# gligen/GLIGEN

Hardware: NVIDIA H100
Metric: 512x512 50-step PLMS box+text images/sec (higher is better)
Workload: dtype bf16

## Files before the change

gligen_b200/csrc/gemm_tc.cu:

```cuda
#include "gemm_tc.cuh"

namespace glg {

__global__ void splitk_reduce_kernel(const GemmKParams p) {
  pdl_trigger();
  pdl_wait();
  const int nv = p.N >> 3;
  const long long total = (long long)p.M * nv;
  const float gate = p.gate ? __ldg(p.gate) : 1.0f;
  for (long long i = (long long)blockIdx.x * blockDim.x + threadIdx.x; i < total; i += (long long)gridDim.x * blockDim.x) {
    const int row = (int)(i / nv), n0 = (int)(i % nv) * 8;
    float v[8] = {0.f, 0.f, 0.f, 0.f, 0.f, 0.f, 0.f, 0.f};
    for (int s = 0; s < p.splits; ++s) {
      const float4* w4 = reinterpret_cast<const float4*>(p.ws + ((size_t)s * p.M + row) * p.N + n0);
      const float4 a = w4[0], b = w4[1];
      v[0] += a.x; v[1] += a.y; v[2] += a.z; v[3] += a.w; v[4] += b.x; v[5] += b.y; v[6] += b.z; v[7] += b.w;
    }
    if (p.bias) {
#pragma unroll
      for (int j = 0; j < 8; ++j) v[j] += __ldg(p.bias + n0 + j);
    }
    if (p.rowbias) {
      const float* rb = p.rowbias + (size_t)(row / p.rows_per_batch) * p.ld_rowbias + n0;
#pragma unroll
      for (int j = 0; j < 8; ++j) v[j] += __ldg(rb + j);
    }
#pragma unroll
    for (int j = 0; j < 8; ++j) v[j] = act_f(p.act, v[j]);
    if (p.gate) {
#pragma unroll
      for (int j = 0; j < 8; ++j) v[j] *= gate;
    }
    if (p.residual) {
      const uint4 u = __ldg(reinterpret_cast<const uint4*>(p.residual + (size_t)row * p.ldr + n0));
      float2 f;
      f = unpack_bf16x2(u.x); v[0] += f.x; v[1] += f.y;
      f = unpack_bf16x2(u.y); v[2] += f.x; v[3] += f.y;
      f = unpack_bf16x2(u.z); v[4] += f.x; v[5] += f.y;
      f = unpack_bf16x2(u.w); v[6] += f.x; v[7] += f.y;
    }
    const size_t out_off = p.orpb ? (size_t)(row / p.orpb) * p.obs + (size_t)(row % p.orpb) * p.ldc : (size_t)row * p.ldc;
    uint4 o;
    o.x = pack_bf16x2(v[0], v[1]); o.y = pack_bf16x2(v[2], v[3]); o.z = pack_bf16x2(v[4], v[5]); o.w = pack_bf16x2(v[6], v[7]);
    *reinterpret_cast<uint4*>(reinterpret_cast<bf16*>(p.out) + out_off + n0) = o;
  }
}

int g_force_bn = 0;
int g_splitk_mode = 0;
int g_cta2_mode = -1;
int g_bres_mode = -1;
int g_pp_mode = 0;

static constexpr long long kTileMax = 227 * 1024 - 1024 - 1024;

static int bres_stages(int bn, int num_kb) {
  const long long left = kTileMax - (long long)num_kb * bn * 128;
  if (left < 3 * 16384) return 0;
  const int st = (int)(left / 16384);
  return st > 12 ? 12 : st;
}

static bool pingpong_pays(int M, int bn, bool geglu, bool conv) {
  return (conv && M >= 8192 && bn == 64) || (geglu && M <= 512);
}

static void pick_tile(int M, int N, int num_kb, bool geglu, bool conv, int max_splits, long long ws_bytes,
                      int* bn_out, int* cta2_out, int* splits_out, int* bres_out, int* pp_out) {
  if (g_cta2_mode < 0) {
    const char* e = getenv("GLG_GEMM_CTA2");
    g_cta2_mode = e ? atoi(e) : 0;
  }
  if (g_bres_mode < 0) {
    const char* e = getenv("GLG_GEMM_BRES");
    g_bres_mode = e ? atoi(e) : 1;
  }
  const int sms = num_sms();
  const int cands[4] = {256, 160, 128, 64};
  float best = 1e30f; int best_bn = 0, best_pair = 0, best_s = 1, best_res = 0, best_pp = 0;
  for (int pair = 0; pair < 2; ++pair) {
    if (pair && (g_cta2_mode == 1 || M <= 128)) continue;
    if (pair && g_cta2_mode == 0 && !conv && (N % 256 || num_kb < 16 || M < 4096)) continue;
    if (pair && g_cta2_mode == 0 && conv && M < 2048) continue;
    if (!pair && g_cta2_mode == 2 && M > 128) {
      bool any = false;
      for (int i = 0; i < 3; ++i) any |= (N % cands[i] == 0) && (!geglu || cands[i] == 256);
      if (any) continue;
    }
    for (int i = 0; i < 4; ++i) {
      const int bn = cands[i];
      if (N % bn) continue;
      if (geglu && bn != 256) continue;
      if (g_force_bn && bn != g_force_bn && (N % g_force_bn == 0) && !geglu) continue;
      if (pair && bn < 128) continue;
      if (pair && g_cta2_mode == 0 && !conv && bn != 256) continue;
      for (int pp = 0; pp < 2; ++pp) {
        if (pp && (g_pp_mode == 1 || (!geglu && bn > 128))) continue;
        if (pp && g_pp_mode == 0 && !pingpong_pays(M, bn, geglu, conv)) continue;
        const int kbn = (pp && geglu) ? 128 : bn;
        const float force = pp ? 1e-3f : 1.0f;
        const int rows = pair ? 256 : 128;
        const int tiles = ((M + rows - 1) / rows) * (N / kbn);
        const int units = pair ? sms / 2 : sms;
        const float mma = 4.0f * kbn;
        const float l2 = 4.0f * (pair ? 128.0f + 0.5f * kbn : 128.0f + kbn);
        const float per_kb = mma > l2 ? mma : l2;
        for (int sp = 1; sp <= (pair ? 1 : max_splits); ++sp) {
          if (sp > 1 && (num_kb / sp < (g_splitk_mode == 2 ? 4 : 16) || (long long)sp * M * N * 4 > ws_bytes)) break;
          if (sp > 1 && tiles * 2 > units && g_splitk_mode != 2) break;
          if (g_splitk_mode == 2 && max_splits > 1 && sp == 1 && num_kb >= 8) continue;
          const int waves = (tiles * sp + units - 1) / units;
          const int kb_cta = (num_kb + sp - 1) / sp;
          float t = (float)waves * (per_kb * kb_cta + 3000.0f);
          if (sp > 1) t += 12000.0f + (float)sp * M * N * 4.0f / (sms * 40.0f);
          const int ctas = (pair ? 2 : 1) * (tiles * sp < units ? tiles * sp : units);
          t *= 1.0f + 0.10f * (1.0f - (float)ctas / (float)sms);
          t *= force;
          if (t < best) { best = t; best_bn = bn; best_pair = pair; best_s = sp; best_res = 0; best_pp = pp; }
        }
        const int tiles_n = N / kbn, tiles_m = (M + 127) / 128;
        if (!pair && !conv && g_bres_mode != 1 && tiles_n <= sms && bres_stages(kbn, num_kb) > 0) {
          const int per_n = sms / tiles_n;
          if (tiles_m >= 2 * per_n || g_bres_mode == 2) {
            const int waves = (tiles_m + per_n - 1) / per_n;
            const float l2a = 4.0f * 128.0f;
            float t = (float)waves * ((mma > l2a ? mma : l2a) * num_kb + 3000.0f) + 4.0f * kbn * num_kb;
            const int ctas = per_n * tiles_n;
            t *= 1.0f + 0.10f * (1.0f - (float)ctas / (float)sms);
            if (g_bres_mode == 2) t = -1.0f / (float)bn / force;
            else t *= force;
            if (t < best) { best = t; best_bn = bn; best_pair = 0; best_s = 1; best_res = 1; best_pp = pp; }
          }
        }
      }
    }
  }
  *bn_out = best_bn; *cta2_out = best_pair; *splits_out = best_s; *bres_out = best_res; *pp_out = best_pp;
}


struct GemmInstance { int bn; bool geglu, cta2, pp; int epi; GemmLaunchFn fn; };
#define GLG_GEMM_TABLE_ROW(BN, GEGLU, CTA2, PP, NS) {BN, GEGLU, CTA2, PP, NS::kEpi, &NS::launch<BN, GEGLU, CTA2, PP>},
static const GemmInstance kGemmInstances[] = {GLG_GEMM_INSTANCES(GLG_GEMM_TABLE_ROW)};

static int bn_launch(int bn, bool geglu, bool pp) { return pp && geglu ? 128 : bn; }

static int epilogue_flags(const GemmKParams& p) {
  if (p.splits > 1) return 0;
  return (p.ln_stats ? EPI_LN : 0) | (p.bias ? EPI_BIAS : 0) | (p.rowbias ? EPI_ROWBIAS : 0) | (p.gate ? EPI_GATE : 0) |
         (p.residual ? EPI_RES : 0) | (p.stats_out ? EPI_STATS : 0) | (p.out_fp32 ? EPI_F32 : 0) | (p.orpb ? EPI_ORPB : 0) |
         (p.act ? EPI_ACT : 0);
}

static const GemmInstance* find_instance(int bn, bool geglu, bool cta2, bool pp, int flags) {
  const GemmInstance* generic = nullptr;
  for (const GemmInstance& g : kGemmInstances) {
    if (g.bn != bn || g.geglu != geglu || g.cta2 != cta2 || g.pp != pp) continue;
    if (g.epi == flags) return &g;
    if (g.epi == EPI_GENERIC) generic = &g;
  }
  return generic;
}
}

using namespace glg;

extern "C" void glg_debug_force_bn(int bn) { glg::g_force_bn = bn; }
extern "C" void glg_debug_pick_tile(int M, int N, int K, int geglu, int conv, int can_split, long long ws_bytes, int* out) {
  int bres = 0, pp = 0;
  glg::pick_tile(M, N, (conv ? 9 : 1) * (K / 64), geglu != 0, conv != 0, can_split ? 8 : 1, ws_bytes, &out[0], &out[1], &out[2], &bres, &pp);
  out[1] |= bres << 8;
}
extern "C" int glg_debug_pick_pingpong(int M, int N, int K, int geglu, int conv, int can_split, long long ws_bytes) {
  int bn, pair, sp, bres, pp = 0;
  glg::pick_tile(M, N, (conv ? 9 : 1) * (K / 64), geglu != 0, conv != 0, can_split ? 8 : 1, ws_bytes, &bn, &pair, &sp, &bres, &pp);
  return pp;
}
extern "C" int glg_debug_epilogue_kind(int M, int N, int K, int geglu, int conv, int can_split, long long ws_bytes, int flags) {
  int bn, pair, sp, bres, pp = 0;
  glg::pick_tile(M, N, (conv ? 9 : 1) * (K / 64), geglu != 0, conv != 0, can_split ? 8 : 1, ws_bytes, &bn, &pair, &sp, &bres, &pp);
  const glg::GemmInstance* g = glg::find_instance(glg::bn_launch(bn, geglu != 0, pp != 0), geglu != 0, pair != 0, pp != 0, sp > 1 ? 0 : flags);
  return g ? g->epi : -1;
}
extern "C" void glg_debug_gemm_pp(int mode) { glg::g_pp_mode = mode; }
extern "C" void glg_debug_gemm_bres(int mode) { glg::g_bres_mode = mode; }
extern "C" void glg_debug_gemm_cta2(int mode) { glg::g_cta2_mode = mode; }
extern "C" void glg_debug_splitk(int mode) { glg::g_splitk_mode = mode; }

extern "C" int glg_gemm(const GlgGemmArgs* a, void* stream) {
  if (!a) return set_error("glg_gemm: null args");
  if (a->K <= 0 || a->K % 64) return set_error("glg_gemm: K must be a positive multiple of 64");
  if (a->M <= 0 || a->N <= 0) return set_error("glg_gemm: M, N must be positive");
  if ((a->lda % 8) || (a->ldc % 8) || (a->residual && (a->ldr % 8))) return set_error("glg_gemm: leading dims must be multiples of 8");
  if (((uintptr_t)a->A | (uintptr_t)a->W | (uintptr_t)a->out | (uintptr_t)a->residual) & 15) return set_error("glg_gemm: pointers must be 16-byte aligned");
  if (a->rowbias && ((a->ld_rowbias % 4) || a->rows_per_batch <= 0)) return set_error("glg_gemm: bad rowbias args");
  if (a->geglu && (a->N % 256 || !a->bias || a->out_fp32)) return set_error("glg_gemm: geglu needs N % 256 == 0, a bias and bf16 output");
  int bn = 0, cta2 = 0, splits = 1, bres = 0, pp = 0;
  const bool can_split = a->splitk_ws && g_splitk_mode != 1 && !a->geglu && !a->ln_stats && !a->stats_out && !a->out_fp32 &&
                         !((uintptr_t)a->splitk_ws & 15);
  pick_tile(a->M, a->N, (a->conv_mode ? 9 : 1) * (a->K / 64), a->geglu != 0, a->conv_mode != 0, can_split ? 8 : 1,
            a->splitk_ws_bytes, &bn, &cta2, &splits, &bres, &pp);
  if (!bn) return set_error("glg_gemm: N must be a multiple of 64");
  const int kbn = bn_launch(bn, a->geglu != 0, pp != 0);
  GemmKParams p;
  memset(&p, 0, sizeof(p));
  const int rows_per_tile = cta2 ? 256 : 128;
  p.M = a->M; p.N = a->N;
  p.kb_per_tap = a->K / 64;
  p.num_kb = a->conv_mode ? 9 * p.kb_per_tap : p.kb_per_tap;
  p.tiles_m = (a->M + rows_per_tile - 1) / rows_per_tile;
  p.tiles_n = a->N / kbn;
  p.conv = a->conv_mode;
  p.out = a->out; p.ldc = a->ldc; p.out_fp32 = a->out_fp32;
  p.bias = a->bias; p.rowbias = a->rowbias; p.ld_rowbias = a->ld_rowbias; p.rows_per_batch = a->rows_per_batch > 0 ? a->rows_per_batch : 1;
  p.act = a->act; p.gate = a->gate; p.residual = reinterpret_cast<const bf16*>(a->residual); p.ldr = a->ldr;
  if (a->ln_stats) {
    if (!a->ln_colsum || a->ln_slots <= 0 || a->conv_mode) return set_error("glg_gemm: LayerNorm fold needs ln_colsum, ln_slots > 0 and a plain GEMM");
    if (((uintptr_t)a->ln_stats & 7) || ((uintptr_t)a->ln_colsum & 15)) return set_error("glg_gemm: ln_stats / ln_colsum alignment");
    if (a->ln_slot_stride > 0 && a->ln_slot_stride < a->M) return set_error("glg_gemm: ln_slot_stride < M");
    p.ln_stats = a->ln_stats; p.ln_slots = a->ln_slots; p.ln_colsum = a->ln_colsum; p.ln_eps = a->ln_eps; p.inv_k = 1.0f / (float)a->K;
  }
  if (a->stats_out) {
    if (a->geglu || a->out_fp32 || a->stats_slots * 32 != a->N || ((uintptr_t)a->stats_out & 7))
      return set_error("glg_gemm: stats_out needs a bf16 non-GEGLU output and stats_slots == N / 32");
    p.stats_out = a->stats_out; p.stats_slots = a->stats_slots;
  }
  if (a->out_rows_per_batch > 0) {
    if (a->out_batch_stride % 8) return set_error("glg_gemm: out_batch_stride must be a multiple of 8");
    p.orpb = a->out_rows_per_batch; p.obs = a->out_batch_stride;
  }
  if (a->bias && ((uintptr_t)a->bias & 15)) return set_error("glg_gemm: bias must be 16-byte aligned");

  p.splits = splits;
  p.ws = splits > 1 ? reinterpret_cast<float*>(a->splitk_ws) : nullptr;
  p.b_res = bres;
  const long long stage_bytes = bres ? 16384 : 128 * 128 + kbn * 128;
  const long long fixed = bres ? (long long)p.num_kb * kbn * 128 : 0;
  long long stages = (kTileMax - fixed) / stage_bytes;
  const int cap = bres ? 12 : 8;
  p.stages = (int)(stages > cap ? cap : stages);
  if (p.stages < 2) return set_error("glg_gemm: internal: shared memory budget");
  const size_t smem = (size_t)(p.stages * stage_bytes + fixed) + 1024 + 1024;
  if (a->stats_out) p.stats_stride = a->stats_slot_stride > 0 ? a->stats_slot_stride : a->M;
  if (a->ln_stats) p.ln_stride = a->ln_slot_stride > 0 ? a->ln_slot_stride : a->M;

  const uint32_t brows = (uint32_t)(cta2 || (pp && a->geglu) ? kbn / 2 : kbn);
  CUtensorMap ta, tb;
  if (a->conv_mode) {
    const int H = a->H, W = a->Wd, B = a->Bn;
    if (H <= 0 || W <= 0 || B <= 0 || (long long)B * H * W != a->M) return set_error("glg_gemm: conv dims do not match M");
    const int HW = H * W;
    p.HW = HW; p.Wd = W;
    const uint64_t dims[4] = {(uint64_t)a->K, (uint64_t)W, (uint64_t)H, (uint64_t)B};
    const uint64_t str[3] = {(uint64_t)a->lda * 2, (uint64_t)a->lda * 2 * W, (uint64_t)a->lda * 2 * HW};
    if (get_tmap_bf16_im2col3x3(&ta, a->A, dims, str, 64, 128)) return -1;
    const uint64_t wd[2] = {(uint64_t)a->K, (uint64_t)a->N * 9};
    const uint64_t ws[1] = {(uint64_t)a->K * 2};
    const uint32_t wb[2] = {64, brows};
    if (get_tmap_bf16(&tb, a->W, 2, wd, ws, wb)) return -1;
  } else {
    const uint64_t dims[2] = {(uint64_t)a->K, (uint64_t)a->M};
    const uint64_t str[1] = {(uint64_t)a->lda * 2};
    const uint32_t box[2] = {64, 128};
    if (get_tmap_bf16(&ta, a->A, 2, dims, str, box)) return -1;
    const uint64_t wd[2] = {(uint64_t)a->K, (uint64_t)a->N};
    const uint64_t ws[1] = {(uint64_t)a->K * 2};
    const uint32_t wb[2] = {64, brows};
    if (get_tmap_bf16(&tb, a->W, 2, wd, ws, wb)) return -1;
  }
  const GemmInstance* inst = find_instance(kbn, a->geglu != 0, cta2 != 0, pp != 0, epilogue_flags(p));
  if (!inst) return set_error("glg_gemm: internal: bad tile");
  cudaStream_t st = reinterpret_cast<cudaStream_t>(stream);
  if (inst->fn(ta, tb, p, smem, st)) return -1;
  if (p.splits > 1) {
    const long long total = (long long)p.M * (p.N / 8);
    long long blocks = (total + 255) / 256;
    if (blocks > 4096) blocks = 4096;
    cudaError_t e = launch_k(splitk_reduce_kernel, dim3((unsigned)blocks), dim3(256), 0, st, 1, p);
    count_launch();
    if (e != cudaSuccess) return set_error(std::string("splitk reduce launch: ") + cudaGetErrorString(e));
    return check_launch("splitk reduce launch");
  }
  return 0;
}
```

gligen_b200/csrc/gemm_tc.cuh:

```cuda
#pragma once
#include <cuda.h>
#include <cuda_runtime.h>
#include <stdio.h>
#include <stdlib.h>
#include <string.h>
#include <string>

#include "common.cuh"
#include "internal.h"
#include "wgmma.cuh"
#include "../../include/gligen_b200.h"

namespace glg {

enum : int {
  EPI_LN = 1, EPI_BIAS = 2, EPI_ROWBIAS = 4, EPI_GATE = 8, EPI_RES = 16, EPI_STATS = 32, EPI_F32 = 64, EPI_ORPB = 128,
  EPI_ACT = 256, EPI_GENERIC = 512,
};

struct GemmKParams {
  int M, N, num_kb, kb_per_tap;
  int tiles_m, tiles_n;
  int conv, HW, Wd;
  void* out; long long ldc; int out_fp32;
  const float* bias; const float* rowbias; long long ld_rowbias; int rows_per_batch;
  int act; const float* gate; const bf16* residual; long long ldr;
  const float* ln_stats; int ln_slots; const float* ln_colsum; float ln_eps; float inv_k;
  float* stats_out; int stats_slots;
  int orpb; long long obs;
  int splits; float* ws;
  int stages;
  int b_res;
  long long stats_stride;
  long long ln_stride;
};

template <int BN, bool CTA2> struct GemmCfg {
  static constexpr int BM = 128, BK = 64;
  static constexpr int THREADS = 384;
  static constexpr int A_BYTES = BM * BK * 2;
  static constexpr int B_BYTES = BN * BK * 2;
  static constexpr int B_HALF = B_BYTES / 2;
  static constexpr int STAGE_BYTES = A_BYTES + B_BYTES;
  static constexpr int MAX_STAGES = 12;
  static constexpr int BAR_BYTES = 1024;
  static constexpr int SMEM_MAX = 227 * 1024;
  static_assert(8 * (2 * MAX_STAGES + 1) <= BAR_BYTES, "barrier area");
  static_assert(B_HALF % 1024 == 0, "each half of the B stage must keep the 1024-byte swizzle alignment");
};

__device__ __forceinline__ void setmaxnreg_dec40() { asm volatile("setmaxnreg.dec.sync.aligned.u32 40;"); }
__device__ __forceinline__ void setmaxnreg_inc232() { asm volatile("setmaxnreg.inc.sync.aligned.u32 232;"); }
__device__ __forceinline__ void named_bar_sync(int id) { asm volatile("bar.sync %0, 256;" ::"r"(id) : "memory"); }
__device__ __forceinline__ void named_bar_arrive(int id) { asm volatile("bar.arrive %0, 256;" ::"r"(id) : "memory"); }

template <int BN> __device__ __forceinline__ int geglu_xrow(int n_blk) { return (n_blk * BN / 256) * 256 + (n_blk * (BN / 2)) % 128; }

__device__ __forceinline__ float act_f(int act, float v) {
  if (act == GLG_ACT_SILU) return silu_f(v);
  if (act == GLG_ACT_GELU) return gelu_erf_f(v);
  if (act == GLG_ACT_QUICK_GELU) return quick_gelu_f(v);
  return v;
}

template <int BN, bool GEGLU, int EPI>
__device__ __forceinline__ void epilogue_tile(const GemmKParams& p, float (&d)[BN / 2], int row_base, int n_blk, float gate, int lane) {
  constexpr bool GEN = (EPI & EPI_GENERIC) != 0, ACT = (EPI & EPI_ACT) != 0;
  const bool has_ln = GEN ? p.ln_stats != nullptr : (EPI & EPI_LN) != 0;
  const bool has_bias = GEN ? p.bias != nullptr : (EPI & EPI_BIAS) != 0;
  const bool has_rowbias = GEN ? p.rowbias != nullptr : (EPI & EPI_ROWBIAS) != 0;
  const bool has_gate = GEN ? p.gate != nullptr : (EPI & EPI_GATE) != 0;
  const bool has_res = GEN ? p.residual != nullptr : (EPI & EPI_RES) != 0;
  const bool has_stats = GEN ? p.stats_out != nullptr : (EPI & EPI_STATS) != 0;
  const bool out_f32 = GEN ? p.out_fp32 != 0 : (EPI & EPI_F32) != 0;
  const bool has_orpb = GEN ? p.orpb != 0 : (EPI & EPI_ORPB) != 0;
  const int cq = 2 * (lane & 3);
  int row[2]; bool row_ok[2]; size_t out_off[2];
  float ln_rstd[2] = {1.f, 1.f}, c1[2] = {0.f, 0.f};
#pragma unroll
  for (int hr = 0; hr < 2; ++hr) {
    row[hr] = row_base + hr * 8;
    row_ok[hr] = row[hr] < p.M;
    out_off[hr] = has_orpb ? (size_t)(row[hr] / p.orpb) * p.obs + (size_t)(row[hr] % p.orpb) * p.ldc : (size_t)row[hr] * p.ldc;
  }
  if (has_ln) {
    const float2* sp = reinterpret_cast<const float2*>(p.ln_stats);
    const int r0 = row_ok[0] ? row[0] : 0, r1 = row_ok[1] ? row[1] : 0;
    float s1[2] = {0.f, 0.f}, s2[2] = {0.f, 0.f};
    for (int i = 0; i < p.ln_slots; ++i) {
      const float2 t0 = __ldg(sp + (size_t)i * p.ln_stride + r0), t1 = __ldg(sp + (size_t)i * p.ln_stride + r1);
      s1[0] += t0.x; s2[0] += t0.y; s1[1] += t1.x; s2[1] += t1.y;
    }
#pragma unroll
    for (int hr = 0; hr < 2; ++hr) {
      const float mu = s1[hr] * p.inv_k;
      ln_rstd[hr] = rsqrtf(fmaxf(s2[hr] * p.inv_k - mu * mu, 0.f) + p.ln_eps);
      c1[hr] = -ln_rstd[hr] * mu;
    }
  }
  if constexpr (GEGLU) {
    constexpr int HALF = BN / 2;
    const int xrow = geglu_xrow<BN>(n_blk);
#pragma unroll
    for (int ch = 0; ch < HALF / 32; ++ch) {
      float2 bx[4], bg[4], cx[4], cg[4];
#pragma unroll
      for (int jj = 0; jj < 4; ++jj) {
        const int wcol = xrow + 32 * ch + 8 * jj + cq;
        bx[jj] = __ldg(reinterpret_cast<const float2*>(p.bias + wcol));
        bg[jj] = __ldg(reinterpret_cast<const float2*>(p.bias + wcol + 128));
        if (has_ln) {
          cx[jj] = __ldg(reinterpret_cast<const float2*>(p.ln_colsum + wcol));
          cg[jj] = __ldg(reinterpret_cast<const float2*>(p.ln_colsum + wcol + 128));
        }
      }
#pragma unroll
      for (int hr = 0; hr < 2; ++hr) {
#pragma unroll
        for (int jj = 0; jj < 4; ++jj) {
          const int j = 4 * ch + jj;
          float bx0 = bx[jj].x, bx1 = bx[jj].y, bg0 = bg[jj].x, bg1 = bg[jj].y;
          if (has_ln) {
            bx0 = fmaf(cx[jj].x, c1[hr], bx0); bx1 = fmaf(cx[jj].y, c1[hr], bx1);
            bg0 = fmaf(cg[jj].x, c1[hr], bg0); bg1 = fmaf(cg[jj].y, c1[hr], bg1);
          }
          const float x0 = fmaf(d[4 * j + 2 * hr], ln_rstd[hr], bx0), x1 = fmaf(d[4 * j + 2 * hr + 1], ln_rstd[hr], bx1);
          const float g0 = fmaf(d[HALF / 2 + 4 * j + 2 * hr], ln_rstd[hr], bg0), g1 = fmaf(d[HALF / 2 + 4 * j + 2 * hr + 1], ln_rstd[hr], bg1);
          if (row_ok[hr])
            *reinterpret_cast<uint32_t*>(reinterpret_cast<bf16*>(p.out) + out_off[hr] + n_blk * HALF + 8 * j + cq) = pack_bf16x2(geglu_f(x0, g0), geglu_f(x1, g1));
        }
      }
    }
  } else {
    const float* rb[2];
#pragma unroll
    for (int hr = 0; hr < 2; ++hr) rb[hr] = (has_rowbias && row_ok[hr]) ? p.rowbias + (size_t)(row[hr] / p.rows_per_batch) * p.ld_rowbias : nullptr;
#pragma unroll
    for (int ch = 0; ch < BN / 32; ++ch) {
      float2 bias[4], cs[4], rbv[2][4];
      uint32_t res[2][4];
#pragma unroll
      for (int jj = 0; jj < 4; ++jj) {
        const int n0 = n_blk * BN + 32 * ch + 8 * jj + cq;
        bias[jj] = has_bias ? __ldg(reinterpret_cast<const float2*>(p.bias + n0)) : make_float2(0.f, 0.f);
        if (has_ln) cs[jj] = __ldg(reinterpret_cast<const float2*>(p.ln_colsum + n0));
#pragma unroll
        for (int hr = 0; hr < 2; ++hr) {
          if (rb[hr]) rbv[hr][jj] = __ldg(reinterpret_cast<const float2*>(rb[hr] + n0));
          if (has_res && row_ok[hr]) res[hr][jj] = __ldg(reinterpret_cast<const unsigned int*>(p.residual + (size_t)row[hr] * p.ldr + n0));
        }
      }
#pragma unroll
      for (int hr = 0; hr < 2; ++hr) {
        float st_sum = 0.f, st_sq = 0.f;
#pragma unroll
        for (int jj = 0; jj < 4; ++jj) {
          const int j = 4 * ch + jj;
          const int n0 = n_blk * BN + 8 * j + cq;
          float v0 = d[4 * j + 2 * hr], v1 = d[4 * j + 2 * hr + 1];
          if (has_ln) {
            v0 = fmaf(v0, ln_rstd[hr], fmaf(cs[jj].x, c1[hr], bias[jj].x));
            v1 = fmaf(v1, ln_rstd[hr], fmaf(cs[jj].y, c1[hr], bias[jj].y));
          } else if (has_bias) { v0 += bias[jj].x; v1 += bias[jj].y; }
          if (rb[hr]) { v0 += rbv[hr][jj].x; v1 += rbv[hr][jj].y; }
          if constexpr (ACT) { v0 = act_f(p.act, v0); v1 = act_f(p.act, v1); }
          if (has_gate) { v0 *= gate; v1 *= gate; }
          if (has_res && row_ok[hr]) {
            const float2 r = unpack_bf16x2(res[hr][jj]);
            v0 += r.x; v1 += r.y;
          }
          if (out_f32) {
            if (row_ok[hr]) *reinterpret_cast<float2*>(reinterpret_cast<float*>(p.out) + out_off[hr] + n0) = make_float2(v0, v1);
          } else {
            const uint32_t pk = pack_bf16x2(v0, v1);
            if (row_ok[hr]) *reinterpret_cast<uint32_t*>(reinterpret_cast<bf16*>(p.out) + out_off[hr] + n0) = pk;
            const float2 f = unpack_bf16x2(pk);
            st_sum += f.x + f.y;
            st_sq = fmaf(f.x, f.x, fmaf(f.y, f.y, st_sq));
          }
        }
        if (has_stats && !out_f32) {
          st_sum += __shfl_xor_sync(0xffffffffu, st_sum, 1); st_sq += __shfl_xor_sync(0xffffffffu, st_sq, 1);
          st_sum += __shfl_xor_sync(0xffffffffu, st_sum, 2); st_sq += __shfl_xor_sync(0xffffffffu, st_sq, 2);
          if ((lane & 3) == 0 && row_ok[hr])
            reinterpret_cast<float2*>(p.stats_out)[(size_t)((n_blk * BN >> 5) + ch) * p.stats_stride + row[hr]] = make_float2(st_sum, st_sq);
        }
      }
    }
  }
}
template <int BN>
__device__ __forceinline__ void epilogue_partial(const GemmKParams& p, const float (&d)[BN / 2], int row_base, int n_blk, int split, int lane) {
#pragma unroll
  for (int hr = 0; hr < 2; ++hr) {
    const int row = row_base + hr * 8;
    if (row >= p.M) continue;
    float* dst = p.ws + ((size_t)split * p.M + row) * p.N + (size_t)n_blk * BN + 2 * (lane & 3);
#pragma unroll
    for (int j = 0; j < BN / 8; ++j) *reinterpret_cast<float2*>(dst + 8 * j) = make_float2(d[4 * j + 2 * hr], d[4 * j + 2 * hr + 1]);
  }
}

template <int BN, bool GEGLU, bool CTA2, bool PP, int EPI>
__device__ __forceinline__ void gemm_tc_body(const CUtensorMap& tmA, const CUtensorMap& tmB, const GemmKParams& p) {
  using Cfg = GemmCfg<BN, CTA2>;
  constexpr int MAXST = Cfg::MAX_STAGES;
  constexpr int ROWS_PER_TILE = CTA2 ? 256 : 128;
  constexpr bool B_SPLIT = GEGLU && PP;
  constexpr bool MAY_SPLIT = EPI == 0 || (EPI & EPI_GENERIC) != 0;
  extern __shared__ uint8_t smem_raw[];
  const uint32_t bar_base = (smem_u32(smem_raw) + 1023u) & ~1023u;
  const uint32_t base = bar_base + Cfg::BAR_BYTES;
  const int STAGES = p.stages;
  const bool bres = !CTA2 && p.b_res != 0;
  const uint32_t stage_bytes = bres ? (uint32_t)Cfg::A_BYTES : (uint32_t)Cfg::STAGE_BYTES;
  const uint32_t bres_base = base + (uint32_t)STAGES * Cfg::A_BYTES;
  auto full_bar = [&](int s) { return bar_base + 8u * s; };
  auto empty_bar = [&](int s) { return bar_base + 8u * (MAXST + s); };
  const uint32_t bfull_bar = bar_base + 8u * (2 * MAXST);
  auto b_row = [&](int n_blk, int q) { return B_SPLIT ? geglu_xrow<BN>(n_blk) + q * 128 : n_blk * BN + q * (BN / 2); };

  pdl_trigger();
  const int warp = threadIdx.x >> 5;
  const int lane = threadIdx.x & 31;
  const int wg = warp >> 2;
  const uint32_t rank = CTA2 ? cluster_ctarank() : 0u;
  const int unit = CTA2 ? (int)(blockIdx.x >> 1) : (int)blockIdx.x;
  const int num_units = CTA2 ? (int)(gridDim.x >> 1) : (int)gridDim.x;

  if (threadIdx.x == 0) {
    constexpr uint32_t releasers = (PP ? 4 : 8) * (CTA2 ? 2 : 1);
    for (int s = 0; s < STAGES; ++s) { mbar_init(full_bar(s), 1); mbar_init(empty_bar(s), releasers); }
    mbar_init(bfull_bar, 1);
    fence_barrier_init();
  }
  if (warp == 0 && lane == 0) { tma_prefetch_desc(&tmA); tma_prefetch_desc(&tmB); }
  if constexpr (CTA2) cluster_sync_all(); else __syncthreads();
  pdl_wait();

  const int total_work = p.tiles_m * p.tiles_n * p.splits;
  const int per_n = bres ? num_units / p.tiles_n : 1;
  auto get_work = [&](int it, int& tile, int& split, int& m_blk, int& n_blk) -> bool {
    if (bres) {
      n_blk = unit % p.tiles_n;
      m_blk = unit / p.tiles_n + it * per_n;
      split = 0;
      tile = m_blk * p.tiles_n + n_blk;
      return m_blk < p.tiles_m;
    }
    const int work = unit + it * num_units;
    if (work >= total_work) return false;
    tile = work / p.splits; split = work - tile * p.splits;
    m_blk = tile / p.tiles_n; n_blk = tile - m_blk * p.tiles_n;
    return true;
  };

  if (wg == 0) {
    setmaxnreg_dec40();
    if (warp == 0) {
      const bool leader = elect_one();
      int stage = 0; uint32_t phase = 0;
      if (bres && leader) {
        const int nblk = unit % p.tiles_n;
        mbar_arrive_expect_tx(bfull_bar, (uint32_t)p.num_kb * Cfg::B_BYTES);
        for (int kb = 0; kb < p.num_kb; ++kb) {
          const uint32_t dst = bres_base + (uint32_t)kb * Cfg::B_BYTES;
          tma_load_2d(dst, &tmB, bfull_bar, kb * 64, b_row(nblk, 0));
          if constexpr (B_SPLIT) tma_load_2d(dst + Cfg::B_HALF, &tmB, bfull_bar, kb * 64, b_row(nblk, 1));
        }
      }
      int tile, split, m_blk, n_blk;
      for (int it = 0; get_work(it, tile, split, m_blk, n_blk); ++it) {
        const int kb_lo = (split * p.num_kb) / p.splits, kb_n = ((split + 1) * p.num_kb) / p.splits - kb_lo;
        const int row0 = m_blk * ROWS_PER_TILE + (int)rank * 128;
        int b0 = 0, y0 = 0, x0 = 0;
        if (p.conv) {
          b0 = row0 / p.HW;
          y0 = (row0 - b0 * p.HW) / p.Wd;
          x0 = row0 - b0 * p.HW - y0 * p.Wd;
        }
        int kb = bres ? kb_lo : kb_lo + (int)(((unsigned)tile * 3u) % (unsigned)kb_n);
        for (int it2 = 0; it2 < kb_n; ++it2, kb = (kb + 1 == kb_lo + kb_n) ? kb_lo : kb + 1) {
          mbar_wait<false>(empty_bar(stage), phase ^ 1u);
          const uint32_t a_dst = base + stage * stage_bytes;
          const uint32_t b_dst = a_dst + Cfg::A_BYTES;
          if (leader) {
            mbar_arrive_expect_tx(full_bar(stage), bres ? Cfg::A_BYTES : Cfg::STAGE_BYTES);
            int ca = kb * 64, cb_off = 0;
            if (p.conv) {
              const int tap = kb / p.kb_per_tap;
              const int cb = kb - tap * p.kb_per_tap;
              const int dy = tap / 3, dx = tap - (tap / 3) * 3;
              tma_load_im2col_4d(a_dst, &tmA, full_bar(stage), cb * 64, x0 - 1, y0 - 1, b0, (uint16_t)dx, (uint16_t)dy);
              ca = cb * 64; cb_off = tap * p.N;
            } else {
              tma_load_2d(a_dst, &tmA, full_bar(stage), kb * 64, row0);
            }
            if constexpr (CTA2) {
              tma_load_2d_mc(b_dst + rank * Cfg::B_HALF, &tmB, full_bar(stage), ca, cb_off + b_row(n_blk, (int)rank), (uint16_t)3);
            } else if (!bres) {
              if constexpr (B_SPLIT) {
                tma_load_2d(b_dst, &tmB, full_bar(stage), ca, cb_off + b_row(n_blk, 0));
                tma_load_2d(b_dst + Cfg::B_HALF, &tmB, full_bar(stage), ca, cb_off + b_row(n_blk, 1));
              } else {
                tma_load_2d(b_dst, &tmB, full_bar(stage), ca, cb_off + n_blk * BN);
              }
            }
          }
          if (++stage == STAGES) { stage = 0; phase ^= 1u; }
        }
      }
    }
  } else {
    setmaxnreg_inc232();
    const int cw = wg - 1;
    constexpr int MH = PP ? 2 : 1;
    const float gate = p.gate ? __ldg(p.gate) : 1.0f;
    uint32_t empty0 = empty_bar(0), empty0_peer = 0;
    if constexpr (CTA2) empty0_peer = mapa_cluster(empty_bar(0), rank ^ 1u);
    if (bres) mbar_wait<false>(bfull_bar, 0);
    int stage = 0; uint32_t phase = 0;
    auto release = [&](int s) {
      if (lane == 0) {
        mbar_arrive(empty0 + 8u * s);
        if constexpr (CTA2) mbar_arrive_cluster(empty0_peer + 8u * s);
      }
    };
    float d[MH][BN / 2];
    int tile, split, m_blk, n_blk;
    for (int it = 0; get_work(it, tile, split, m_blk, n_blk); ++it) {
      const int kb_n = ((split + 1) * p.num_kb) / p.splits - (split * p.num_kb) / p.splits;
      if (PP && (it & 1) != cw) {
        stage += kb_n;
        while (stage >= STAGES) { stage -= STAGES; phase ^= 1u; }
        continue;
      }
      if (PP && it > 0) named_bar_sync(1 + cw);
      int prev = -1;
      for (int kb = 0; kb < kb_n; ++kb) {
        mbar_wait<false>(full_bar(stage), phase);
        const uint32_t a_addr = base + stage * stage_bytes + (uint32_t)(PP ? 0 : cw) * (64 * 128);
        const uint64_t bdesc = gmma_desc_kmajor_sw128(bres ? bres_base + (uint32_t)kb * Cfg::B_BYTES : base + stage * stage_bytes + Cfg::A_BYTES);
#pragma unroll
        for (int mh = 0; mh < MH; ++mh) wgmma_fence_regs(d[mh]);
        wgmma_fence();
#pragma unroll
        for (int k = 0; k < 4; ++k) {
#pragma unroll
          for (int mh = 0; mh < MH; ++mh)
            Wgmma<BN>::mma(d[mh], gmma_desc_kmajor_sw128(a_addr + (uint32_t)mh * (64 * 128)) + 2 * k, bdesc + 2 * k, (kb | k) != 0 ? 1 : 0);
        }
        wgmma_commit();
        wgmma_wait<1>();
#pragma unroll
        for (int mh = 0; mh < MH; ++mh) wgmma_fence_regs(d[mh]);
        if (prev >= 0) release(prev);
        prev = stage;
        if (++stage == STAGES) { stage = 0; phase ^= 1u; }
      }
      if constexpr (PP) {
        int t2, s2, m2, n2;
        if (get_work(it + 1, t2, s2, m2, n2)) named_bar_arrive(2 - cw);
      }
      wgmma_wait<0>();
#pragma unroll
      for (int mh = 0; mh < MH; ++mh) wgmma_fence_regs(d[mh]);
      if (prev >= 0) release(prev);
#pragma unroll
      for (int mh = 0; mh < MH; ++mh) {
        const int row_base = m_blk * ROWS_PER_TILE + (int)rank * 128 + (PP ? mh : cw) * 64 + (warp & 3) * 16 + (lane >> 2);
        if (MAY_SPLIT && p.splits > 1) epilogue_partial<BN>(p, d[mh], row_base, n_blk, split, lane);
        else if constexpr ((EPI & EPI_GENERIC) != 0) {
          if (!GEGLU && p.act) epilogue_tile<BN, GEGLU, EPI | EPI_ACT>(p, d[mh], row_base, n_blk, gate, lane);
          else epilogue_tile<BN, GEGLU, EPI>(p, d[mh], row_base, n_blk, gate, lane);
        } else {
          epilogue_tile<BN, GEGLU, EPI>(p, d[mh], row_base, n_blk, gate, lane);
        }
      }
    }
  }
  if constexpr (CTA2) cluster_sync_all();
}

#define GLG_GEMM_EPI_KINDS(X)                                                  \
  X(epi_generic, EPI_GENERIC)                                                  \
  X(epi_none, 0)                                                               \
  X(epi_bias, EPI_BIAS)                                                        \
  X(epi_bias_act, EPI_BIAS | EPI_ACT)                                          \
  X(epi_bias_f32, EPI_BIAS | EPI_F32)                                          \
  X(epi_bias_rowbias, EPI_BIAS | EPI_ROWBIAS)                                  \
  X(epi_bias_res, EPI_BIAS | EPI_RES)                                          \
  X(epi_bias_stats, EPI_BIAS | EPI_STATS)                                      \
  X(epi_bias_res_stats, EPI_BIAS | EPI_RES | EPI_STATS)                        \
  X(epi_bias_gate_res_stats, EPI_BIAS | EPI_GATE | EPI_RES | EPI_STATS)        \
  X(epi_ln_bias, EPI_LN | EPI_BIAS)                                            \
  X(epi_ln_bias_orpb, EPI_LN | EPI_BIAS | EPI_ORPB)

template <int BN, bool CTA2, typename Kern>
int launch_gemm_grid(Kern kern, const CUtensorMap& ta, const CUtensorMap& tb, const GemmKParams& p, size_t smem, cudaStream_t st) {
  const int tiles = p.tiles_m * p.tiles_n * p.splits;
  int grid;
  if (p.b_res) {
    grid = (num_sms() / p.tiles_n) * p.tiles_n;
  } else if (CTA2) {
    const int pairs = num_sms() / 2;
    grid = 2 * (tiles < pairs ? tiles : pairs);
  } else {
    grid = tiles < num_sms() ? tiles : num_sms();
  }
  cudaError_t e = launch_k(kern, dim3(grid), dim3(GemmCfg<BN, CTA2>::THREADS), smem, st, CTA2 ? 2 : 1, ta, tb, p);
  count_launch();
  if (e != cudaSuccess) return set_error(std::string("gemm launch: ") + cudaGetErrorString(e));
  return check_launch("gemm launch");
}

using GemmLaunchFn = int (*)(const CUtensorMap&, const CUtensorMap&, const GemmKParams&, size_t, cudaStream_t);

#define GLG_GEMM_DECLARE_KIND(NS, EPI_BITS)                                                                              \
  namespace NS {                                                                                                         \
  constexpr int kEpi = EPI_BITS;                                                                                         \
  template <int BN, bool GEGLU, bool CTA2, bool PP>                                                                      \
  int launch(const CUtensorMap& ta, const CUtensorMap& tb, const GemmKParams& p, size_t smem, cudaStream_t st);          \
  }
GLG_GEMM_EPI_KINDS(GLG_GEMM_DECLARE_KIND)

#ifdef GLG_GEMM_KERNEL_UNIT
#define GLG_GEMM_DEFINE_KIND(NS, EPI_BITS)                                                                               \
  namespace NS {                                                                                                         \
  template <int BN, bool GEGLU, bool CTA2, bool PP>                                                                      \
  __global__ void __launch_bounds__(384, 1)                                                                              \
  gemm_tc_kernel(const __grid_constant__ CUtensorMap tmA, const __grid_constant__ CUtensorMap tmB, const GemmKParams p) { \
    gemm_tc_body<BN, GEGLU, CTA2, PP, kEpi>(tmA, tmB, p);                                                                \
  }                                                                                                                      \
  template <int BN, bool GEGLU, bool CTA2, bool PP>                                                                      \
  int launch(const CUtensorMap& ta, const CUtensorMap& tb, const GemmKParams& p, size_t smem, cudaStream_t st) {         \
    static bool attr_set = false;                                                                                        \
    auto kern = gemm_tc_kernel<BN, GEGLU, CTA2, PP>;                                                                     \
    if (!attr_set) {                                                                                                     \
      cudaError_t e = cudaFuncSetAttribute(kern, cudaFuncAttributeMaxDynamicSharedMemorySize, GemmCfg<BN, CTA2>::SMEM_MAX); \
      if (e != cudaSuccess) return set_error(std::string("cudaFuncSetAttribute(gemm): ") + cudaGetErrorString(e));       \
      attr_set = true;                                                                                                   \
    }                                                                                                                    \
    return launch_gemm_grid<BN, CTA2>(kern, ta, tb, p, smem, st);                                                        \
  }                                                                                                                      \
  }
GLG_GEMM_EPI_KINDS(GLG_GEMM_DEFINE_KIND)
#endif

#define GLG_GEMM_GENERIC(X, BN, GEGLU, CTA2, PP) X(BN, GEGLU, CTA2, PP, epi_generic)
#define GLG_GEMM_UNET_COOP(X, BN)                                                                                          \
  X(BN, false, false, false, epi_none) X(BN, false, false, false, epi_bias) X(BN, false, false, false, epi_bias_f32)      \
  X(BN, false, false, false, epi_bias_res) X(BN, false, false, false, epi_bias_stats)                                     \
  X(BN, false, false, false, epi_bias_res_stats) X(BN, false, false, false, epi_bias_gate_res_stats)                      \
  X(BN, false, false, false, epi_ln_bias) X(BN, false, false, false, epi_ln_bias_orpb)
#define GLG_GEMM_CONV(X, BN, CTA2, PP)                                                                                     \
  X(BN, false, CTA2, PP, epi_bias) X(BN, false, CTA2, PP, epi_bias_rowbias) X(BN, false, CTA2, PP, epi_bias_res)

#define GLG_GEMM_INSTANCES_BN64(X)                                                                                         \
  GLG_GEMM_GENERIC(X, 64, false, false, false) GLG_GEMM_GENERIC(X, 64, false, false, true)                                \
  GLG_GEMM_UNET_COOP(X, 64) X(64, false, false, false, epi_bias_act) X(64, false, false, false, epi_bias_rowbias)         \
  GLG_GEMM_CONV(X, 64, false, true)
#define GLG_GEMM_INSTANCES_BN128(X)                                                                                        \
  GLG_GEMM_GENERIC(X, 128, false, false, false) GLG_GEMM_GENERIC(X, 128, false, true, false)                              \
  GLG_GEMM_GENERIC(X, 128, false, false, true) GLG_GEMM_GENERIC(X, 128, false, true, true)                                \
  GLG_GEMM_GENERIC(X, 128, true, false, true) GLG_GEMM_GENERIC(X, 128, true, true, true)                                  \
  GLG_GEMM_UNET_COOP(X, 128) GLG_GEMM_CONV(X, 128, true, false) X(128, true, false, true, epi_ln_bias)
#define GLG_GEMM_INSTANCES_BN160(X)                                                                                        \
  GLG_GEMM_GENERIC(X, 160, false, false, false) GLG_GEMM_GENERIC(X, 160, false, true, false)                              \
  GLG_GEMM_UNET_COOP(X, 160) GLG_GEMM_CONV(X, 160, true, false)
#define GLG_GEMM_INSTANCES_BN256(X)                                                                                        \
  GLG_GEMM_GENERIC(X, 256, false, false, false) GLG_GEMM_GENERIC(X, 256, false, true, false)                              \
  GLG_GEMM_GENERIC(X, 256, true, false, false) GLG_GEMM_GENERIC(X, 256, true, true, false)                                \
  X(256, false, false, false, epi_none) X(256, false, false, false, epi_bias) X(256, false, false, false, epi_bias_act)    \
  X(256, false, false, false, epi_bias_stats) X(256, false, false, false, epi_ln_bias)                                    \
  X(256, false, false, false, epi_ln_bias_orpb)                                                                           \
  X(256, false, true, false, epi_bias) X(256, false, true, false, epi_bias_f32) X(256, false, true, false, epi_bias_stats) \
  X(256, false, true, false, epi_ln_bias) X(256, false, true, false, epi_ln_bias_orpb)                                    \
  X(256, true, false, false, epi_ln_bias) X(256, true, true, false, epi_ln_bias)
#define GLG_GEMM_INSTANCES(X)                                                                                              \
  GLG_GEMM_INSTANCES_BN64(X) GLG_GEMM_INSTANCES_BN128(X) GLG_GEMM_INSTANCES_BN160(X) GLG_GEMM_INSTANCES_BN256(X)

#define GLG_GEMM_INSTANTIATE(BN, GEGLU, CTA2, PP, NS)                                                                    \
  template int NS::launch<BN, GEGLU, CTA2, PP>(const CUtensorMap&, const CUtensorMap&, const GemmKParams&, size_t, cudaStream_t);

}
```

Before: 2.452.

## Move ping-pong GEMM to BN=160 large-M tiles and drop conv-specific instances

Changes the tile-selection heuristic so ping-pong warpgroup scheduling targets BN=160 tiles with large M (non-geglu) instead of BN=64 conv tiles, disables 2-CTA pairs for conv, and adds BN=160 ping-pong instantiations across the epilogues. A fallback to the non-pingpong instance covers missing variants. The ping-pong mainloop now explicitly zeroes accumulators per tile, and the residual epilogue precomputes per-row residual pointers. It aims to overlap epilogue and MMA on the large UNet GEMMs. Removing the conv 2-CTA and BN=64 ping-pong paths could slow conv layers.

```diff
diff --git a/gligen_b200/csrc/gemm_tc.cu b/gligen_b200/csrc/gemm_tc.cu
--- a/gligen_b200/csrc/gemm_tc.cu
+++ b/gligen_b200/csrc/gemm_tc.cu
@@ -61,9 +61,7 @@
   return st > 12 ? 12 : st;
 }
 
-static bool pingpong_pays(int M, int bn, bool geglu, bool conv) {
-  return (conv && M >= 8192 && bn == 64) || (geglu && M <= 512);
-}
+static bool pingpong_pays(int M, int bn, bool geglu) { return geglu ? M <= 512 : bn == 160 && M >= 8192; }
 
 static void pick_tile(int M, int N, int num_kb, bool geglu, bool conv, int max_splits, long long ws_bytes,
                       int* bn_out, int* cta2_out, int* splits_out, int* bres_out, int* pp_out) {
@@ -81,7 +79,7 @@
   for (int pair = 0; pair < 2; ++pair) {
     if (pair && (g_cta2_mode == 1 || M <= 128)) continue;
     if (pair && g_cta2_mode == 0 && !conv && (N % 256 || num_kb < 16 || M < 4096)) continue;
-    if (pair && g_cta2_mode == 0 && conv && M < 2048) continue;
+    if (pair && g_cta2_mode == 0 && conv) continue;
     if (!pair && g_cta2_mode == 2 && M > 128) {
       bool any = false;
       for (int i = 0; i < 3; ++i) any |= (N % cands[i] == 0) && (!geglu || cands[i] == 256);
@@ -95,10 +93,10 @@
       if (pair && bn < 128) continue;
       if (pair && g_cta2_mode == 0 && !conv && bn != 256) continue;
       for (int pp = 0; pp < 2; ++pp) {
-        if (pp && (g_pp_mode == 1 || (!geglu && bn > 128))) continue;
-        if (pp && g_pp_mode == 0 && !pingpong_pays(M, bn, geglu, conv)) continue;
+        if (pp && (g_pp_mode == 1 || (!geglu && bn > 160))) continue;
+        if (pp && g_pp_mode == 0 && !pingpong_pays(M, bn, geglu)) continue;
         const int kbn = (pp && geglu) ? 128 : bn;
-        const float force = pp ? 1e-3f : 1.0f;
+        const float force = pp ? (g_pp_mode == 2 ? 1e-3f : 0.999f) : 1.0f;
         const int rows = pair ? 256 : 128;
         const int tiles = ((M + rows - 1) / rows) * (N / kbn);
         const int units = pair ? sms / 2 : sms;
@@ -179,7 +177,9 @@
 extern "C" int glg_debug_epilogue_kind(int M, int N, int K, int geglu, int conv, int can_split, long long ws_bytes, int flags) {
   int bn, pair, sp, bres, pp = 0;
   glg::pick_tile(M, N, (conv ? 9 : 1) * (K / 64), geglu != 0, conv != 0, can_split ? 8 : 1, ws_bytes, &bn, &pair, &sp, &bres, &pp);
-  const glg::GemmInstance* g = glg::find_instance(glg::bn_launch(bn, geglu != 0, pp != 0), geglu != 0, pair != 0, pp != 0, sp > 1 ? 0 : flags);
+  const int kbn = glg::bn_launch(bn, geglu != 0, pp != 0);
+  const glg::GemmInstance* g = glg::find_instance(kbn, geglu != 0, pair != 0, pp != 0, sp > 1 ? 0 : flags);
+  if (!g && pp && !geglu) g = glg::find_instance(kbn, false, pair != 0, false, sp > 1 ? 0 : flags);
   return g ? g->epi : -1;
 }
 extern "C" void glg_debug_gemm_pp(int mode) { glg::g_pp_mode = mode; }
@@ -269,6 +269,7 @@
     if (get_tmap_bf16(&tb, a->W, 2, wd, ws, wb)) return -1;
   }
   const GemmInstance* inst = find_instance(kbn, a->geglu != 0, cta2 != 0, pp != 0, epilogue_flags(p));
+  if (!inst && pp && !a->geglu) inst = find_instance(kbn, false, cta2 != 0, false, epilogue_flags(p));
   if (!inst) return set_error("glg_gemm: internal: bad tile");
   cudaStream_t st = reinterpret_cast<cudaStream_t>(stream);
   if (inst->fn(ta, tb, p, smem, st)) return -1;
diff --git a/gligen_b200/csrc/gemm_tc.cuh b/gligen_b200/csrc/gemm_tc.cuh
--- a/gligen_b200/csrc/gemm_tc.cuh
+++ b/gligen_b200/csrc/gemm_tc.cuh
@@ -133,8 +133,12 @@
     }
   } else {
     const float* rb[2];
-#pragma unroll
-    for (int hr = 0; hr < 2; ++hr) rb[hr] = (has_rowbias && row_ok[hr]) ? p.rowbias + (size_t)(row[hr] / p.rows_per_batch) * p.ld_rowbias : nullptr;
+    const bf16* rr[2];
+#pragma unroll
+    for (int hr = 0; hr < 2; ++hr) {
+      rb[hr] = (has_rowbias && row_ok[hr]) ? p.rowbias + (size_t)(row[hr] / p.rows_per_batch) * p.ld_rowbias : nullptr;
+      rr[hr] = has_res ? p.residual + (size_t)row[hr] * p.ldr + n_blk * BN + cq : nullptr;
+    }
 #pragma unroll
     for (int ch = 0; ch < BN / 32; ++ch) {
       float2 bias[4], cs[4], rbv[2][4];
@@ -147,7 +151,7 @@
 #pragma unroll
         for (int hr = 0; hr < 2; ++hr) {
           if (rb[hr]) rbv[hr][jj] = __ldg(reinterpret_cast<const float2*>(rb[hr] + n0));
-          if (has_res && row_ok[hr]) res[hr][jj] = __ldg(reinterpret_cast<const unsigned int*>(p.residual + (size_t)row[hr] * p.ldr + n0));
+          if (has_res && row_ok[hr]) res[hr][jj] = __ldg(reinterpret_cast<const unsigned int*>(rr[hr] + 32 * ch + 8 * jj));
         }
       }
 #pragma unroll
@@ -336,6 +340,12 @@
         continue;
       }
       if (PP && it > 0) named_bar_sync(1 + cw);
+      if constexpr (PP) {
+#pragma unroll
+        for (int mh = 0; mh < MH; ++mh)
+#pragma unroll
+          for (int i = 0; i < BN / 2; ++i) d[mh][i] = 0.f;
+      }
       int prev = -1;
       for (int kb = 0; kb < kb_n; ++kb) {
         mbar_wait<false>(full_bar(stage), phase);
@@ -453,21 +463,22 @@
   X(BN, false, false, false, epi_bias_res) X(BN, false, false, false, epi_bias_stats)                                     \
   X(BN, false, false, false, epi_bias_res_stats) X(BN, false, false, false, epi_bias_gate_res_stats)                      \
   X(BN, false, false, false, epi_ln_bias) X(BN, false, false, false, epi_ln_bias_orpb)
-#define GLG_GEMM_CONV(X, BN, CTA2, PP)                                                                                     \
-  X(BN, false, CTA2, PP, epi_bias) X(BN, false, CTA2, PP, epi_bias_rowbias) X(BN, false, CTA2, PP, epi_bias_res)
-
 #define GLG_GEMM_INSTANCES_BN64(X)                                                                                         \
   GLG_GEMM_GENERIC(X, 64, false, false, false) GLG_GEMM_GENERIC(X, 64, false, false, true)                                \
-  GLG_GEMM_UNET_COOP(X, 64) X(64, false, false, false, epi_bias_act) X(64, false, false, false, epi_bias_rowbias)         \
-  GLG_GEMM_CONV(X, 64, false, true)
+  GLG_GEMM_UNET_COOP(X, 64) X(64, false, false, false, epi_bias_act) X(64, false, false, false, epi_bias_rowbias)
 #define GLG_GEMM_INSTANCES_BN128(X)                                                                                        \
   GLG_GEMM_GENERIC(X, 128, false, false, false) GLG_GEMM_GENERIC(X, 128, false, true, false)                              \
   GLG_GEMM_GENERIC(X, 128, false, false, true) GLG_GEMM_GENERIC(X, 128, false, true, true)                                \
   GLG_GEMM_GENERIC(X, 128, true, false, true) GLG_GEMM_GENERIC(X, 128, true, true, true)                                  \
-  GLG_GEMM_UNET_COOP(X, 128) GLG_GEMM_CONV(X, 128, true, false) X(128, true, false, true, epi_ln_bias)
+  GLG_GEMM_UNET_COOP(X, 128) X(128, true, false, true, epi_ln_bias)
+#define GLG_GEMM_PP160(X)                                                                                                  \
+  X(160, false, false, true, epi_bias) X(160, false, false, true, epi_bias_f32) X(160, false, false, true, epi_bias_rowbias) \
+  X(160, false, false, true, epi_bias_res) X(160, false, false, true, epi_bias_stats)                                     \
+  X(160, false, false, true, epi_bias_res_stats) X(160, false, false, true, epi_bias_gate_res_stats)                      \
+  X(160, false, false, true, epi_ln_bias) X(160, false, false, true, epi_ln_bias_orpb)
 #define GLG_GEMM_INSTANCES_BN160(X)                                                                                        \
   GLG_GEMM_GENERIC(X, 160, false, false, false) GLG_GEMM_GENERIC(X, 160, false, true, false)                              \
-  GLG_GEMM_UNET_COOP(X, 160) GLG_GEMM_CONV(X, 160, true, false)
+  GLG_GEMM_UNET_COOP(X, 160) X(160, false, false, false, epi_bias_rowbias) GLG_GEMM_PP160(X)
 #define GLG_GEMM_INSTANCES_BN256(X)                                                                                        \
   GLG_GEMM_GENERIC(X, 256, false, false, false) GLG_GEMM_GENERIC(X, 256, false, true, false)                              \
   GLG_GEMM_GENERIC(X, 256, true, false, false) GLG_GEMM_GENERIC(X, 256, true, true, false)                                \
```

Measured after the change: 2.698 (median of 6 runs). 10.0% higher.
